# simon3dv/SLR-SFS

Hardware: AMD Instinct MI355X
Metric: synthesised frames/sec at 768x1280 N=60 (higher is better)
Workload: dtype f32 (convs: fp32 in/out/accumulate, operands 2 x f16 splits = 22 bits; all-fp32: fps_fp32_convs); 1 GPU; C3 baseline pipeline, 768x1280, N=60, random weights; parallelism=1 GPU, no collective, collective_bytes_received_per_rank_per_clip=0

## Files before the change

### slr-sfs_amd/csrc/conv.hip

```cpp
#include "slr_common.hpp"

#include <string.h>

#include <atomic>
#include <mutex>
#include <type_traits>

namespace slr {

typedef _Float16 h8 __attribute__((ext_vector_type(8)));
typedef float f16v __attribute__((ext_vector_type(16)));

constexpr int CV_W = 32, CV_H = 8;
constexpr int CV_HW = CV_W + 2, CV_HH = CV_H + 2;
constexpr int CV_NPX = CV_HW * CV_HH;
constexpr int CV_THREADS = 256;
constexpr float CV_XSCALE = 64.0f;
constexpr int CV_MAXCIN = 1024;

enum { PRE_NONE = 0, PRE_BN = 1, PRE_BN_MASK = 2, PRE_BN_NONZERO = 3 };

struct ConvArgs {
    const float *in;
    const h8 *w;
    float *out;
    int N, Cin, Cout, H, W, tiles_x, nchunk;
    float unscale;
    float xscale;
    int pre;
    const float *pre_scale, *pre_shift;
    const float *mask;
    const float *bias;
    int partial;
    float mask_scale, winsize;
    const float *residual, *next_scale, *next_shift;
    float *um_out;
    int out_b8;
    int res_b8;
    unsigned *sat;
#ifdef SLR_TRACE
    long long *trace;
#endif
    int wino_groups;
    const float *skip_in;
    const h8 *skip_w;
    const float *skip_bias;
    int skip_cin, skip_nchunk;
    float skip_unscale;
    float *pool_row, *pool_col;
    int tiles_y, resample;
    float *skip_out;
};

__host__ __device__ inline int conv_cout_tile(int Cout) { return Cout > 64 ? 128 : (Cout > 32 ? 64 : 32); }
__host__ __device__ inline int conv_cout_pad(int Cout) { const int t = conv_cout_tile(Cout); return (Cout + t - 1) / t * t; }
__host__ __device__ inline int conv_cin_pad(int Cin) { return (Cin + 15) / 16 * 16; }

}
#include "conv_few.hpp"
namespace slr {

constexpr int CV_FSTR = 352;
constexpr int CV_KSTR = 260;
template <int CPW, int WCO, bool PRE, bool INB8, bool F32 = false, bool SKIP = false, bool POOL = false, bool UPS = false>
__global__ __launch_bounds__(CV_THREADS, 2) void conv3x3_split_kernel(ConvArgs a) {
    constexpr int WPX = 4 / WCO, PT = CV_H / WPX;
    static_assert(!(POOL || UPS) || (SKIP && WCO == 4 && !(POOL && UPS)), "the resampling epilogues: a wave holds all 8 rows of its channel tile");
    static_assert(!F32 || CPW == 1, "the fp32 rung runs one 32-channel tile per wave");
    static_assert(!SKIP || (CPW == 1 && INB8), "the skip phase: one tile per wave, channel-blocked main input");
    constexpr int XRAW = F32 ? 2 * 16 * CV_FSTR * 4 : 2 * 2 * 2 * CV_NPX * 16, XSKIP = !SKIP ? 0 : SLR_CONV_SKIP_FILL * (F32 ? 16 * CV_KSTR * 4 : 2 * 2 * 256 * 16);
    __shared__ __attribute__((aligned(16))) unsigned char xraw[XRAW > XSKIP ? XRAW : XSKIP];
    h8 (*xs)[2][2][CV_NPX] = reinterpret_cast<h8 (*)[2][2][CV_NPX]>(xraw);
    float (*xf)[16][CV_FSTR] = reinterpret_cast<float (*)[16][CV_FSTR]>(xraw);
    __shared__ float mpl[CV_NPX];
    __shared__ float mplB[2][CV_NPX - 256];
    __shared__ float4 pss4[2][CV_MAXCIN / 4];
    const int tid = threadIdx.x, lane = tid & 63;
    const int wave = __builtin_amdgcn_readfirstlane(tid >> 6);
    const int wc = wave % WCO, wp = wave / WCO;
    const int tx = blockIdx.x % a.tiles_x, ty = blockIdx.x / a.tiles_x;
    const int x0 = tx * CV_W, y0 = ty * CV_H;
    const int n = blockIdx.z;
    const int cot0 = (blockIdx.y * WCO + wc) * CPW;
    const int HW = a.H * a.W;
    const int nchunk = a.nchunk;
    const int cmax = a.Cin - 1;
    const float *inb = a.in + (size_t)n * a.Cin * HW;
    const int pre = a.pre;

    if (PRE) {
        float *pssw = reinterpret_cast<float *>(&pss4[0][0]);
        for (int i = tid; i < nchunk * 16; i += CV_THREADS) {
            pssw[i] = i < a.Cin ? a.pre_scale[i] * (F32 ? 1.0f : a.xscale) : 0.0f;
            pssw[CV_MAXCIN + i] = i < a.Cin ? a.pre_shift[i] * (F32 ? 1.0f : a.xscale) : 0.0f;
        }
    }

    const int gB = tid >= 84 ? 1 : 0;
    const int pB = 256 + tid - 84 * gB;
    const bool liveB = tid < 168;
    bool okA, okB;
    int offA, offB;
    {
        const int pr = tid / CV_HW, pc = tid - pr * CV_HW;
        const int gy = y0 - 1 + pr, gx = x0 - 1 + pc;
        okA = (gy >= 0) & (gy < a.H) & (gx >= 0) & (gx < a.W);
        offA = okA ? gy * a.W + gx : 0;
    }
    {
        const int pr = pB / CV_HW, pc = pB - pr * CV_HW;
        const int gy = y0 - 1 + pr, gx = x0 - 1 + pc;
        okB = liveB & (gy >= 0) & (gy < a.H) & (gx >= 0) & (gx < a.W);
        offB = okB ? gy * a.W + gx : 0;
    }
    const float unit = (PRE || F32) ? 1.0f : a.xscale;
    const float mvA = (a.mask && okA) ? a.mask[(size_t)n * HW + offA] : 0.0f;
    const float mvB = (a.mask && okB) ? a.mask[(size_t)n * HW + offB] : 0.0f;
    if (a.mask) {
        mpl[tid] = mvA;
        if (tid < CV_NPX - 256) mpl[256 + tid] = mvB;
    }
    const float mA = okA ? (pre == PRE_BN_MASK ? mvA : unit) : 0.0f;
    const float mB = okB ? (pre == PRE_BN_MASK ? mvB : unit) : 0.0f;
    float cnt[3] = {0.0f, 0.0f, 0.0f};
    const bool nonzero_mask = pre == PRE_BN_NONZERO;
    const int c8max = (a.Cin >> 3) - 1;
    auto load_round = [&](auto R, int c, float (&st)[8]) {
        if (INB8) {
            const int grp = min(c * 2 + (R.value < 2 ? R.value : gB), c8max);
            const float4 *q = reinterpret_cast<const float4 *>(inb) + ((size_t)grp * HW + (unsigned)(R.value < 2 ? offA : offB)) * 2;
            const float4 u = q[0], v = q[1];
            st[0] = u.x; st[1] = u.y; st[2] = u.z; st[3] = u.w;
            st[4] = v.x; st[5] = v.y; st[6] = v.z; st[7] = v.w;
            return;
        }
#pragma unroll
        for (int j = 0; j < 8; ++j) {
            if (R.value < 2) {
                const float *pl = inb + (size_t)min(c * 16 + R.value * 8 + j, cmax) * HW;
                st[j] = pl[(unsigned)offA];
            } else {
                st[j] = inb[(unsigned)(min(c * 16 + gB * 8 + j, cmax) * HW + offB)];
            }
        }
    };
    struct Stage { int cb; float mk0, fresh, cnt; h8 hi, lo; float f[F32 ? 8 : 1]; };
    unsigned long long sat = 0ull;
    const float *pss = reinterpret_cast<const float *>(&pss4[0][0]);
    auto stage_begin = [&](auto R, int c, Stage &g) {
        g.cb = c * 16 + (R.value < 2 ? R.value * 8 : gB * 8);
        g.mk0 = R.value < 2 ? mA : mB;
        g.cnt = 0.0f;
    };
    auto stage_value = [&](int j, Stage &g, const float (&st)[8], const float *psc = nullptr, const float *psh = nullptr) {
        const float x = st[j];
        float v;
        if (PRE) {
            const float mk = (nonzero_mask & (x == 0.0f)) ? 0.0f : g.mk0;
            v = fmaxf(x * (psc ? psc[j] : pss[g.cb + j]) - (psh ? psh[j] : pss[CV_MAXCIN + g.cb + j]), 0.0f) * mk;
            g.cnt += (g.cb + j <= cmax) ? mk : 0.0f;
        } else if (F32) {
            v = g.mk0 != 0.0f ? x : 0.0f;
        } else {
            v = x * g.mk0;
        }
        if (F32) { g.f[j] = v; return; }
// ... 185 lines not shown
#pragma unroll
            for (int ct = 0; ct < CPW; ++ct) {
                a_cur[ct][0] = a_nxt[ct][0]; a_cur[ct][1] = a_nxt[ct][1];
                if (DEEP) { a_nxt[ct][0] = a_nx2[ct][0]; a_nxt[ct][1] = a_nx2[ct][1]; }
            }
        }
        __syncthreads();
    }

    if (pre == PRE_BN_NONZERO) {
        mpl[tid] = cnt[0] + cnt[1];
        if (liveB) mplB[gB][pB - 256] = cnt[2];
        __syncthreads();
        if (tid < CV_NPX - 256) mpl[256 + tid] = mplB[0][tid] + mplB[1][tid];
    }
    __syncthreads();

    if constexpr (SKIP) {
        constexpr int SK = SLR_CONV_SKIP_FILL;
        static_assert(SK * (F32 ? 16 * CV_KSTR * 4 : 2 * 2 * 256 * 16) <= (int)sizeof(xraw), "skip fills live in the staging buffers");
        h8 (*xk)[2][2][256] = reinterpret_cast<h8 (*)[2][2][256]>(xraw);
        float (*xkf)[16][CV_KSTR] = reinterpret_cast<float (*)[16][CV_KSTR]>(xraw);
        const int ns = a.skip_nchunk, sc8max = (a.skip_cin >> 3) - 1;
        const int spr = tid >> 5, spc = tid & 31;
        const bool sok = (y0 + spr < a.H) & (x0 + spc < a.W);
        const float smk = sok ? a.xscale : 0.0f;
        const float4 *sq = reinterpret_cast<const float4 *>(a.skip_in + (size_t)n * a.skip_cin * HW) + (size_t)(sok ? (y0 + spr) * a.W + x0 + spc : 0) * 2;
        float4 sv[SK][4];
        auto sload = [&](int s0) {
#pragma unroll
            for (int k = 0; k < SK; ++k)
#pragma unroll
                for (int g = 0; g < 2; ++g) {
                    const float4 *q = sq + (size_t)min(min(s0 + k, ns - 1) * 2 + g, sc8max) * HW * 2;
                    sv[k][2 * g] = q[0];
                    sv[k][2 * g + 1] = q[1];
                }
        };
        auto sstore = [&]() {
#pragma unroll
            for (int k = 0; k < SK; ++k)
#pragma unroll
                for (int g = 0; g < 2; ++g) {
                    const float x8[8] = {sv[k][2 * g].x, sv[k][2 * g].y, sv[k][2 * g].z, sv[k][2 * g].w,
                                         sv[k][2 * g + 1].x, sv[k][2 * g + 1].y, sv[k][2 * g + 1].z, sv[k][2 * g + 1].w};
                    if constexpr (F32) {
#pragma unroll
                        for (int j = 0; j < 8; ++j) xkf[k][8 * g + j][tid] = x8[j] * smk;
                        continue;
                    }
                    h8 hi, lo;
#pragma unroll
                    for (int j = 0; j < 8; ++j) {
                        const float v = __builtin_amdgcn_fmed3f(x8[j] * smk, -65472.0f, 65472.0f);
                        sat |= __ballot(fabsf(v) >= 65472.0f);
                        const _Float16 h = (_Float16)v;
                        hi[j] = h;
                        lo[j] = (_Float16)(v - (float)h);
                    }
                    xk[k][0][g][tid] = hi;
                    xk[k][1][g][tid] = lo;
                }
        };
        sload(0);
        {
            const bool partial = a.partial != 0, has_bias = a.bias != nullptr;
            const float unscale = a.unscale, rescale = 1.0f / a.skip_unscale;
            const float mscale = a.mask_scale, winsize = a.winsize;
            float eb[16];
#pragma unroll
            for (int r = 0; r < 16; ++r) eb[r] = has_bias ? a.bias[min(cot0 * 32 + (r & 3) + 8 * (r >> 2) + 4 * (lane >> 5), a.Cout - 1)] : 0.0f;
#pragma unroll
            for (int pt = 0; pt < PT; ++pt) {
                if (partial) {
                    float box = 0.0f;
#pragma unroll
                    for (int dy = 0; dy < 3; ++dy)
#pragma unroll
                        for (int dx = 0; dx < 3; ++dx) box += mpl[(wp * PT + pt + dy) * CV_HW + (lane & 31) + dx];
                    const float u = box * mscale;
                    const float um = F32 ? clamp01_nan(u) : fminf(fmaxf(u, 0.0f), 1.0f);
                    const float ratio = (1.0f / (u + 1e-8f)) * winsize * um;
                    const int oy = y0 + wp * PT + pt, ox = x0 + (lane & 31);
                    if (ox < a.W && oy < a.H && a.um_out && blockIdx.y == 0 && wc == 0 && lane < 32)
                        a.um_out[(size_t)n * HW + (size_t)oy * a.W + ox] = um;
#pragma unroll
                    for (int r = 0; r < 16; ++r) acc[0][pt][r] = (((acc[0][pt][r] * unscale) * ratio + eb[r]) * um) * rescale;
                } else {
#pragma unroll
                    for (int r = 0; r < 16; ++r) acc[0][pt][r] = (acc[0][pt][r] * unscale + eb[r]) * rescale;
                }
            }
        }
        const h8 *swbase = a.skip_w + (size_t)cot0 * ((size_t)ns * 128);
        for (int s0 = 0; s0 < ns; s0 += SK) {
            sstore();
            h8 sa[SK][2];
#pragma unroll
            for (int k = 0; k < SK; ++k) {
                const h8 *q = swbase + (size_t)min(s0 + k, ns - 1) * 128;
                if (F32) { sa[k][0] = q[2u * (unsigned)lane]; sa[k][1] = q[2u * (unsigned)lane + 1u]; continue; }
                sa[k][0] = q[(unsigned)lane]; sa[k][1] = q[(unsigned)lane + 64u];
            }
            __syncthreads();
            sload(s0 + SK);
            __builtin_amdgcn_sched_barrier(0);
#pragma unroll
            for (int k = 0; k < SK; ++k) {
                if (s0 + k >= ns) break;
                if constexpr (F32) {
                    typedef float f8v __attribute__((ext_vector_type(8)));
                    union AW { h8 h[2]; f8v f; } aw;
                    aw.h[0] = sa[k][0]; aw.h[1] = sa[k][1];
#pragma unroll
                    for (int kp = 0; kp < 8; ++kp) {
                        float bv[PT];
#pragma unroll
                        for (int kk = 0; kk < PT; ++kk) bv[kk] = xkf[k][kp + 8 * (lane >> 5)][(wp * PT + kk) * 32 + (lane & 31)];
#pragma unroll
                        for (int kk = 0; kk < PT; ++kk) acc[0][kk] = __builtin_amdgcn_mfma_f32_32x32x2f32(aw.f[kp], bv[kk], acc[0][kk], 0, 0, 0);
                    }
                    continue;
                }
                const h8 *xh = &xk[k][0][lane >> 5][0], *xl = &xk[k][1][lane >> 5][0];
                constexpr int PB = PT > 4 ? 4 : PT, NB = PT / PB;
#pragma unroll
                for (int hb = 0; hb < NB; ++hb) {
                    h8 bh[PB], bl[PB];
#pragma unroll
                    for (int kk = 0; kk < PB; ++kk) {
                        const int p = (wp * PT + hb * PB + kk) * 32 + (lane & 31);
                        bh[kk] = xh[p];
                        bl[kk] = xl[p];
                    }
#pragma unroll
                    for (int part = 0; part < 3; ++part)
#pragma unroll
                        for (int kk = 0; kk < PB; ++kk)
                            acc[0][hb * PB + kk] = __builtin_amdgcn_mfma_f32_32x32x16_f16(part == 0 ? sa[k][1] : sa[k][0], part == 1 ? bl[kk] : bh[kk],
                                                                                          acc[0][hb * PB + kk], 0, 0, 0);
                }
            }
            __syncthreads();
        }
    }

    if (!F32 && a.sat && sat != 0ull && lane == 0) atomicAdd(a.sat, 1u);

    if constexpr (POOL) {
        const float unscale = a.skip_unscale;
        const int ox = x0 + bcol;
        const bool xin = ox < a.W;
        const int OH = (a.H - 1) / 2 + 1, OW = (a.W - 1) / 2 + 1, C8 = a.Cout >> 3;
        float sb[16];
#pragma unroll
        for (int r = 0; r < 16; ++r) sb[r] = a.skip_bias ? a.skip_bias[min(cot0 * 32 + (r & 3) + 8 * (r >> 2) + 4 * bgrp, a.Cout - 1)] : 0.0f;
#pragma unroll
        for (int pt = 0; pt < PT; ++pt) {
            const bool ok = xin & (y0 + pt < a.H);
#pragma unroll
            for (int r = 0; r < 16; ++r) acc[0][pt][r] = ok ? acc[0][pt][r] * unscale + sb[r] : 0.0f;
        }
#pragma unroll
        for (int q = 0; q < 4; ++q) {
            const int c8 = cot0 * 4 + q;
            if (c8 * 8 + 4 * bgrp >= a.Cout) continue;
            if (xin && y0 + 7 < a.H) {
                float *rb = a.pool_row + ((((size_t)n * a.tiles_y + ty) * C8 + c8) * a.W + ox) * 8 + 4 * bgrp;
// ... 65 lines not shown
            }
        }
#pragma unroll
        for (int pt = 1; pt < PT; ++pt)
            if (y0 + pt >= a.H) {
#pragma unroll
                for (int r = 0; r < 16; ++r) acc[0][pt][r] = acc[0][pt - 1][r];
            }
#pragma unroll
        for (int q = 0; q < 4; ++q) {
            const int c8 = cot0 * 4 + q;
            float hE[PT][4], hO[PT][4];
#pragma unroll
            for (int pt = 0; pt < PT; ++pt)
#pragma unroll
                for (int e = 0; e < 4; ++e) {
                    const float v = acc[0][pt][4 * q + e];
                    const float left = __shfl_up(v, 1, 32), rgt = __shfl_down(v, 1, 32);
                    hE[pt][e] = 0.25f * left + 0.75f * v;
                    hO[pt][e] = 0.75f * v + 0.25f * (rclamp ? v : rgt);
                }
            if (!xin || c8 * 8 + 4 * bgrp >= a.Cout) continue;
            float *ob = a.out + (((size_t)n * C8 + c8) * OH * OW + (size_t)(2 * y0) * OW + 2 * ox) * 8 + 4 * bgrp;
#pragma unroll
            for (int hr = 1; hr < 2 * PT - 1; ++hr) {
                const int ra = (hr & 1) ? hr >> 1 : (hr >> 1) - 1, rb = ra + 1;
                const float l0 = (hr & 1) ? 0.75f : 0.25f, l1 = (hr & 1) ? 0.25f : 0.75f;
                if (y0 + (hr >> 1) >= a.H) continue;
                float *orow = ob + (size_t)hr * OW * 8;
                if (bcol > 0)
                    *reinterpret_cast<float4 *>(orow) = make_float4(l0 * hE[ra][0] + l1 * hE[rb][0], l0 * hE[ra][1] + l1 * hE[rb][1],
                                                                    l0 * hE[ra][2] + l1 * hE[rb][2], l0 * hE[ra][3] + l1 * hE[rb][3]);
                if (bcol < 31)
                    *reinterpret_cast<float4 *>(orow + 8) = make_float4(l0 * hO[ra][0] + l1 * hO[rb][0], l0 * hO[ra][1] + l1 * hO[rb][1],
                                                                        l0 * hO[ra][2] + l1 * hO[rb][2], l0 * hO[ra][3] + l1 * hO[rb][3]);
            }
        }
        return;
    }

    const float *ebias = SKIP ? a.skip_bias : a.bias;
    const bool partial = !SKIP && a.partial != 0, has_bias = ebias != nullptr, has_res = a.residual != nullptr,
               has_next = !SKIP && a.next_scale != nullptr;
    float *outp = a.out;
    const bool vec = !a.out_b8 && (a.W % 4 == 0) && (x0 + CV_W <= a.W) &&
                     !(((uintptr_t)a.out | (uintptr_t)a.residual) & 15);
    constexpr int SCR_STRIDE = 36;
    float *scr = reinterpret_cast<float *>(xraw) + wave * (32 * SCR_STRIDE);
    const int ox = x0 + bcol;
    const bool xin_img = ox < a.W;
    const int cout1 = a.Cout - 1;
    const float mscale = a.mask_scale, winsize = a.winsize, unscale = SKIP ? a.skip_unscale : a.unscale;
#pragma unroll
    for (int ct = 0; ct < CPW; ++ct) {
        int co[16];
#pragma unroll
        for (int r = 0; r < 16; ++r) co[r] = (cot0 + ct) * 32 + (r & 3) + 8 * (r >> 2) + 4 * bgrp;
        float eb[16], esc[16], esh[16];
        if (has_bias) {
#pragma unroll
            for (int r = 0; r < 16; ++r) eb[r] = ebias[min(co[r], cout1)];
        }
        if (has_next) {
#pragma unroll
            for (int r = 0; r < 16; ++r) { esc[r] = a.next_scale[min(co[r], cout1)]; esh[r] = a.next_shift[min(co[r], cout1)]; }
        }
#pragma unroll
        for (int pt = 0; pt < PT; ++pt) {
            const int oy = y0 + wp * PT + pt;
            const bool ok = xin_img & (oy < a.H);
            const size_t pix = ok ? (size_t)oy * a.W + ox : 0;
            float o[16];
#pragma unroll
            for (int r = 0; r < 16; ++r) o[r] = acc[ct][pt][r] * unscale;
            if (partial) {
                float box = 0.0f;
#pragma unroll
                for (int dy = 0; dy < 3; ++dy)
#pragma unroll
                    for (int dx = 0; dx < 3; ++dx) box += mpl[(wp * PT + pt + dy) * CV_HW + bcol + dx];
                const float u = box * mscale;
                const float um = F32 ? clamp01_nan(u) : fminf(fmaxf(u, 0.0f), 1.0f);
                const float ratio = (1.0f / (u + 1e-8f)) * winsize * um;
                if (ok && a.um_out && ct == 0 && blockIdx.y == 0 && wc == 0 && bgrp == 0)
                    a.um_out[(size_t)n * HW + pix] = um;
#pragma unroll
                for (int r = 0; r < 16; ++r) o[r] = (o[r] * ratio + eb[r]) * um;
                if (has_res && !vec && !a.out_b8) {
                    float rv[16];
#pragma unroll
                    for (int r = 0; r < 16; ++r) rv[r] = a.residual[((size_t)n * a.Cout + min(co[r], cout1)) * HW + pix];
#pragma unroll
                    for (int r = 0; r < 16; ++r) o[r] += rv[r];
                }
                if (has_next) {
#pragma unroll
                    for (int r = 0; r < 16; ++r) o[r] = fmaxf(o[r] * esc[r] - esh[r], 0.0f) * um;
                }
            } else {
                if (has_bias) {
#pragma unroll
                    for (int r = 0; r < 16; ++r) o[r] += eb[r];
                }
                if (has_res && !vec && !a.out_b8) {
                    float rv[16];
#pragma unroll
                    for (int r = 0; r < 16; ++r) rv[r] = a.residual[((size_t)n * a.Cout + min(co[r], cout1)) * HW + pix];
#pragma unroll
                    for (int r = 0; r < 16; ++r) o[r] += rv[r];
                }
            }
            if (a.out_b8) {
#pragma unroll
                for (int q = 0; q < 4; ++q) {
                    const int c8 = (cot0 + ct) * 4 + q;
                    const bool live = ok && c8 * 8 + 4 * bgrp < a.Cout;
                    const size_t bidx = (((size_t)n * (a.Cout >> 3) + (live ? c8 : 0)) * HW + pix) * 8 + 4 * bgrp;
                    float4 v = make_float4(o[4 * q], o[4 * q + 1], o[4 * q + 2], o[4 * q + 3]);
                    if (has_res) {
                        float4 rv;
                        if (a.res_b8) {
                            rv = *reinterpret_cast<const float4 *>(&a.residual[bidx]);
                        } else {
                            const size_t ridx = ((size_t)n * a.Cout + (live ? c8 * 8 + 4 * bgrp : 0)) * HW + pix;
                            rv = make_float4(a.residual[ridx], a.residual[ridx + HW], a.residual[ridx + 2 * (size_t)HW], a.residual[ridx + 3 * (size_t)HW]);
                        }
                        v.x += rv.x; v.y += rv.y; v.z += rv.z; v.w += rv.w;
                    }
                    if (live) *reinterpret_cast<float4 *>(&outp[bidx]) = v;
                }
            } else if (vec) {
#pragma unroll
                for (int r = 0; r < 16; ++r) scr[((r & 3) + 8 * (r >> 2) + 4 * bgrp) * SCR_STRIDE + bcol] = o[r];
                __builtin_amdgcn_wave_barrier();
                const int quad = lane & 7;
                float4 v[4], rv[4];
#pragma unroll
                for (int k = 0; k < 4; ++k) v[k] = *reinterpret_cast<const float4 *>(&scr[((lane >> 3) + 8 * k) * SCR_STRIDE + quad * 4]);
                __builtin_amdgcn_wave_barrier();
                const bool rowok = oy < a.H;
                size_t vidx[4];
#pragma unroll
                for (int k = 0; k < 4; ++k) {
                    const int cv = min((cot0 + ct) * 32 + (lane >> 3) + 8 * k, cout1);
                    vidx[k] = ((size_t)n * a.Cout + cv) * HW + (rowok ? (size_t)oy * a.W + x0 + quad * 4 : 0);
                }
                if (has_res) {
#pragma unroll
                    for (int k = 0; k < 4; ++k) rv[k] = *reinterpret_cast<const float4 *>(&a.residual[vidx[k]]);
#pragma unroll
                    for (int k = 0; k < 4; ++k) { v[k].x += rv[k].x; v[k].y += rv[k].y; v[k].z += rv[k].z; v[k].w += rv[k].w; }
                }
#pragma unroll
                for (int k = 0; k < 4; ++k)
                    if (rowok && (cot0 + ct) * 32 + (lane >> 3) + 8 * k <= cout1) *reinterpret_cast<float4 *>(&outp[vidx[k]]) = v[k];
            } else {
#pragma unroll
                for (int r = 0; r < 16; ++r)
                    if (ok && co[r] <= cout1) outp[((size_t)n * a.Cout + co[r]) * HW + pix] = o[r];
            }
        }
    }
}

constexpr int C1_TILES = 1;
template <int NCT, bool INB8, bool F32 = false>
__global__ __launch_bounds__(256) void conv1x1_split_kernel(const float *__restrict__ in, const h8 *__restrict__ w,
                                                            const float *__restrict__ bias, float *__restrict__ out,
                                                            int Cin, int Cout, int HW, int nchunk, float unscale, float xscale,
                                                            int out_b8, unsigned *__restrict__ sat_count) {
    const int lane = threadIdx.x & 63;
    const int wave = __builtin_amdgcn_readfirstlane(threadIdx.x >> 6);
    const int n = blockIdx.z;
    const int cot0 = blockIdx.y * NCT;
    const int pcol = lane & 31, grp = lane >> 5;
    const int p0 = ((blockIdx.x * 4 + wave) * C1_TILES) * 32 + pcol;
    const int cmax = Cin - 1;
    const int gend = C1_TILES * nchunk;
    const float *inb = in + (size_t)n * Cin * HW;
    auto load_x = [&](float (&x)[8], int g) {
        g = min(g, gend - 1);
        const int t = g / nchunk, c = g - t * nchunk;
        const int p = p0 + t * 32;
        const unsigned poff = p < HW ? p : 0;
        if (INB8) {
            const float4 *q4 = reinterpret_cast<const float4 *>(inb) + ((size_t)min(c * 2 + grp, (Cin >> 3) - 1) * HW + poff) * 2;
            const float4 u = q4[0], v = q4[1];
            x[0] = u.x; x[1] = u.y; x[2] = u.z; x[3] = u.w; x[4] = v.x; x[5] = v.y; x[6] = v.z; x[7] = v.w;
            return;
        }
#pragma unroll
        for (int j = 0; j < 8; ++j) x[j] = inb[(size_t)min(c * 16 + grp * 8 + j, cmax) * HW + poff];
    };
    const h8 *wb = w + (size_t)cot0 * nchunk * 128 + lane;
    auto load_a = [&](h8 (&d)[NCT][2], int g) {
        const int c = g % nchunk;
#pragma unroll
        for (int t = 0; t < NCT; ++t) {
            const h8 *q = wb + ((size_t)t * nchunk + c) * 128;
            if (F32) { d[t][0] = q[lane]; d[t][1] = q[lane + 1]; continue; }
            d[t][0] = q[0];
            d[t][1] = q[64];
        }
    };
    const int cout1 = Cout - 1;
    const bool has_bias = bias != nullptr;
    const float *bp = has_bias ? bias : in;
    f16v acc[NCT];
    float x0[8], x1[8], x2[8];
    h8 a_cur[NCT][2], a_nxt[NCT][2];
    bool sat = false;
    load_x(x0, 0);
    load_a(a_cur, 0);
    load_x(x1, 1);
    for (int tile = 0, g = 0; tile < C1_TILES; ++tile) {
        const int p = p0 + tile * 32;
        const bool ok = p < HW;
        const float okf = ok ? xscale : 0.0f;
#pragma unroll
        for (int t = 0; t < NCT; ++t)
#pragma unroll
            for (int r = 0; r < 16; ++r) acc[t][r] = 0.0f;
        for (int c = 0; c < nchunk; ++c, ++g) {
            load_a(a_nxt, g + 1);
            load_x(x2, g + 2);
            __builtin_amdgcn_sched_barrier(0);
            if constexpr (F32) {
                typedef float f8v __attribute__((ext_vector_type(8)));
                const float ok1 = ok ? 1.0f : 0.0f;
#pragma unroll
                for (int kp = 0; kp < 8; ++kp)
#pragma unroll
                    for (int t = 0; t < NCT; ++t) {
                        union AW { h8 h[2]; f8v f; } aw;
                        aw.h[0] = a_cur[t][0]; aw.h[1] = a_cur[t][1];
                        acc[t] = __builtin_amdgcn_mfma_f32_32x32x2f32(aw.f[kp], x0[kp] * ok1, acc[t], 0, 0, 0);
                    }
#pragma unroll
                for (int j = 0; j < 8; ++j) { x0[j] = x1[j]; x1[j] = x2[j]; }
#pragma unroll
                for (int t = 0; t < NCT; ++t) { a_cur[t][0] = a_nxt[t][0]; a_cur[t][1] = a_nxt[t][1]; }
                continue;
// ... 500 lines not shown
        SLR_CHECK_ARG(!sb8 && !pool, "layout flags");
        SLR_CHECK_ARG(sk->w && a.Cout <= CF_MAXCO && (layout & SLR_CONV_IN_B8) && !((uintptr_t)sk->w & 15),
                      "the skip output needs Cout <= 4, a channel-blocked input and 16-byte aligned [Cin][4] weights");
        SLR_CHECK_ARG(a.pre != PRE_BN_NONZERO, "the skip output goes with an explicit mask");
        a.skip_w = (const h8 *)sk->w; a.skip_bias = sk->bias; a.skip_out = sk->skip_out;
        return 0;
    }
    SLR_CHECK_ARG(sk->in && sk->w, "null pointer");
    SLR_CHECK_ARG(!(layout & SLR_CONV_WINO), "no fused skip branch in the Winograd kernel");
    SLR_CHECK_ARG(!(layout & SLR_CONV_F32) || (conv_cout_tile(a.Cout) == 128 && sk->wscale == 1.0f),
                  "the fused skip branch on the fp32 rung: more than 64 output channels, skip_wscale = 1");
    SLR_CHECK_ARG((layout & SLR_CONV_IN_B8) && a.Cout > CF_MAXCO, "the fused skip branch needs a channel-blocked main input and more than 4 output channels");
    SLR_CHECK_ARG(sk->cin > 0 && (long long)sk->cin * a.H * a.W < (1LL << 31) && sk->wscale > 0.0f, "skip sizes");
    SLR_CHECK_ARG(sb8 && sk->cin % 8 == 0 && !((uintptr_t)sk->in & 15), "the fused skip branch reads a channel-blocked skip input (SLR_CONV_SKIP_B8): skip_cin % 8 == 0, 16-byte aligned");
    SLR_CHECK_ARG(!a.residual && !a.next_scale, "the fused skip branch replaces the residual; no next-BN fusion with it");
    a.skip_in = sk->in; a.skip_w = (const h8 *)sk->w; a.skip_bias = sk->bias;
    a.skip_cin = sk->cin; a.skip_nchunk = conv_cin_pad(sk->cin) / 16;
    a.skip_unscale = 1.0f / (xscale * sk->wscale);
    if (pool) {
        SLR_CHECK_ARG(!(up && (layout_in & SLR_CONV_POOL_OUT)), "SLR_CONV_POOL_OUT and SLR_CONV_UP_OUT are exclusive");
        SLR_CHECK_ARG(a.out_b8 && conv_cout_tile(a.Cout) == 128, "the resampling epilogues need a channel-blocked output and more than 64 output channels");
        SLR_CHECK_ARG(!up || (long long)a.N * a.Cout * a.H * a.W < (1LL << 38), "sizes");
        SLR_CHECK_ARG(sk->pool_ws && !((uintptr_t)sk->pool_ws & 15) && sk->pool_ws_bytes >= conv_pool_ws_bytes(a.N, a.Cout, a.H, a.W, up),
                      "pool_ws: slr_conv_pool_ws_bytes / slr_conv_up_ws_bytes, 16-byte aligned");
        a.tiles_y = (a.H + CV_H - 1) / CV_H;
        a.resample = up ? 2 : 1;
        a.pool_row = (float *)sk->pool_ws;
        a.pool_col = a.pool_row + (size_t)a.N * a.Cout * a.tiles_y * a.W * (up ? 2 : 1);
    }
    return 0;
}

template <int WCO, bool PRE, bool B8, bool F32, bool SKIP, bool POOL, bool UPS>
static constexpr bool conv_split_built() {
    return !(WCO == 4 && PRE && !B8) && (B8 || !SKIP) && (!(POOL || UPS) || (SKIP && WCO == 4 && !(POOL && UPS))) &&
           !(F32 && SKIP && WCO != 4);
}

static int conv_launch(ConvArgs &a, float wscale, float xscale, int layout, hipStream_t st) {
    const bool in_b8 = (layout & SLR_CONV_IN_B8) != 0, f32 = (layout & SLR_CONV_F32) != 0, wino = (layout & SLR_CONV_WINO) != 0;
    const bool pre = a.pre != PRE_NONE;
    if (int e = check_xscale(xscale)) return e;
    SLR_CHECK_ARG(!f32 || (wscale == 1.0f && xscale == 1.0f), "the fp32 rung takes no operand scales (wscale = xscale = 1)");
    SLR_CHECK_ARG(!wino || (f32 && a.Cout > CF_MAXCO), "SLR_CONV_WINO goes with SLR_CONV_F32 and more than 4 output channels");
    SLR_CHECK_ARG(!wino || !pre || a.Cin <= WN_MAXCIN, "SLR_CONV_WINO with a prologue supports Cin <= 256");
    if (wino) {
        a.tiles_x = (a.W + WN_BW - 1) / WN_BW;
        a.nchunk = conv_cin_pad(a.Cin) / 16;
        a.xscale = 1.0f; a.unscale = 1.0f;
        const int blocks = a.tiles_x * ((a.H + WN_BH - 1) / WN_BH), ngrp = wino_cout_pad(a.Cout) / 64;
        const dim3 grid((blocks + WN_SLICE - 1) / WN_SLICE * WN_SLICE * ngrp, 1, a.N);
        a.wino_groups = ngrp;
#ifdef SLR_TRACE
        a.trace = g_trace;
#endif
        if (int e = dispatch([&](auto pre_, auto b8) {
                static LdsOptIn attr;
                if (int e = lds_opt_in((const void *)conv3x3_wino_kernel<pre_, b8>, (int)WN_LDS_BYTES, attr)) return e;
                hipLaunchKernelGGL((conv3x3_wino_kernel<pre_, b8>), grid, dim3(WN_THREADS), WN_LDS_BYTES, st, a);
                return 0;
            }, pre, in_b8)) return e;
        SLR_CHECK_LAUNCH();
        return 0;
    }
    if (a.Cout <= CF_MAXCO) {
        const dim3 grid(((a.W + CF_BW - 1) / CF_BW) * ((a.H + CF_BH - 1) / CF_BH), 1, a.N);
        if (int e = dispatch_int<1, 2, 3, 4>(a.Cout, [&](auto nco) {
                return dispatch([&](auto pre_, auto b8, auto skp) {
                    if constexpr (b8 || !skp) hipLaunchKernelGGL((conv3x3_few_kernel<nco, pre_, b8, skp>), grid, dim3(CF_THREADS), 0, st, a);
                    else return conv_not_built();
                    return 0;
                }, pre, in_b8, a.skip_out != nullptr);
            })) return e;
        SLR_CHECK_LAUNCH();
        return 0;
    }
    a.tiles_x = (a.W + CV_W - 1) / CV_W;
    a.nchunk = conv_cin_pad(a.Cin) / 16;
    a.xscale = xscale;
    a.unscale = 1.0f / (xscale * wscale);
    if (int e = sat_counter(&a.sat)) return e;
    int ct = conv_cout_tile(a.Cout);
    if (ct == 128 && pre && !in_b8) ct = 64;
    const dim3 grid(a.tiles_x * ((a.H + CV_H - 1) / CV_H), conv_cout_pad(a.Cout) / ct, a.N);
    if (int e = dispatch_int<4, 2, 1>(ct / 32, [&](auto wco) {
            return dispatch([&](auto pre_, auto b8, auto f32_, auto skip, auto pool, auto ups) {
                if constexpr (conv_split_built<wco, pre_, b8, f32_, skip, pool, ups>())
                    hipLaunchKernelGGL((conv3x3_split_kernel<1, wco, pre_, b8, f32_, skip, pool, ups>), grid, dim3(CV_THREADS), 0, st, a);
                else return conv_not_built();
                return 0;
            }, pre, in_b8, f32, a.skip_in != nullptr, a.resample == 1, a.resample == 2);
        })) return e;
    SLR_CHECK_LAUNCH();
    if (a.resample == 2) {
        const int items = 2 * a.tiles_y * 2 * a.W + 2 * a.tiles_x * 2 * a.H;
        hipLaunchKernelGGL(upsample_fix_kernel, dim3((items + 255) / 256, a.N * (a.Cout >> 3)), dim3(256), 0, st, a.out, (const float *)a.pool_row,
                           (const float *)a.pool_col, a.Cout >> 3, a.H, a.W, a.tiles_x, a.tiles_y);
        SLR_CHECK_LAUNCH();
    } else if (a.resample == 1) {
        const int OH = (a.H - 1) / 2 + 1, OW = (a.W - 1) / 2 + 1;
        const int items = (a.tiles_y - 1) * OW + (a.tiles_x - 1) * OH;
        if (items > 0) {
            hipLaunchKernelGGL(pool_fix_kernel, dim3((items + 255) / 256, a.N * (a.Cout >> 3)), dim3(256), 0, st, a.out, (const float *)a.pool_row,
                               (const float *)a.pool_col, a.Cout >> 3, a.H, a.W, a.tiles_x, a.tiles_y);
            SLR_CHECK_LAUNCH();
        }
    }
    return 0;
}

static int conv3x3_run(bool partial, const float *x, const float *pre_scale, const float *pre_shift, const float *mask,
                       const void *wsplit, float wscale, float xscale, const float *bias, const float *residual,
                       const float *next_scale, const float *next_shift, float *out, float *um_out,
                       int N, int Cin, int Cout, int H, int W, const SkipOp *sk, int layout, void *stream) {
    SLR_CHECK_ARG(x && wsplit && (bias || !partial) && out, "null pointer");
    if (int e = conv_check_layout(layout, x, out, Cin, Cout, residual, partial && !mask)) return e;
    SLR_CHECK_ARG(!pre_scale == !pre_shift, "pre_scale / pre_shift go together");
    SLR_CHECK_ARG(!pre_scale || Cin <= CV_MAXCIN, "prologue supports Cin <= 1024");
    SLR_CHECK_ARG(!partial || mask || pre_scale, "mask = NULL (derived from x != 0) needs the raw input, i.e. pre_scale / pre_shift");
    SLR_CHECK_ARG(!next_scale == !next_shift, "next_scale / next_shift go together");
    SLR_CHECK_ARG(!(residual && next_scale), "residual and next-BN fusion are exclusive");
    if (int e = conv_check_dims(N, Cin, Cout, H, W)) return e;
    ConvArgs a = {};
    a.in = x; a.w = (const h8 *)wsplit; a.bias = bias; a.out = out;
    a.N = N; a.Cin = Cin; a.Cout = Cout; a.H = H; a.W = W;
    a.pre = !pre_scale ? PRE_NONE : !partial ? PRE_BN : mask ? PRE_BN_MASK : PRE_BN_NONZERO;
    a.pre_scale = pre_scale; a.pre_shift = pre_shift; a.mask = mask;
    if (partial) {
        a.partial = 1;
        a.mask_scale = mask ? (float)Cin : 1.0f;
        a.winsize = (float)Cin * 9.0f;
    }
    a.residual = residual; a.next_scale = next_scale; a.next_shift = next_shift; a.um_out = um_out;
    a.out_b8 = (layout & SLR_CONV_OUT_B8) != 0;
    a.res_b8 = (layout & SLR_CONV_RES_B8) != 0;
    if (int e = conv_set_skip(a, sk, xscale, layout)) return e;
    return conv_launch(a, wscale, xscale, layout, (hipStream_t)stream);
}

SLR_EXPORT int slr_conv3x3_forward(const float *in, const void *wsplit, const float *bias, const float *residual,
                                   float *out, int N, int Cin, int Cout, int H, int W, float wscale, float xscale,
                                   const float *pre_scale, const float *pre_shift, int layout, void *stream) {
    return conv3x3_run(false, in, pre_scale, pre_shift, nullptr, wsplit, wscale, xscale, bias, residual, nullptr, nullptr, out, nullptr,
                       N, Cin, Cout, H, W, nullptr, layout, stream);
}

SLR_EXPORT int slr_conv3x3_forward_skip(const float *in, const void *wsplit, const float *bias, float *out,
                                        int N, int Cin, int Cout, int H, int W, float wscale, float xscale,
                                        const float *pre_scale, const float *pre_shift,
                                        const float *skip_in, const void *skip_wsplit, const float *skip_bias, int skip_cin, float skip_wscale,
                                        void *pool_ws, size_t pool_ws_bytes, int layout, void *stream) {
    const SkipOp sk = {skip_in, skip_wsplit, skip_bias, skip_cin, skip_wscale, pool_ws, pool_ws_bytes, nullptr};
    return conv3x3_run(false, in, pre_scale, pre_shift, nullptr, wsplit, wscale, xscale, bias, nullptr, nullptr, nullptr, out, nullptr,
                       N, Cin, Cout, H, W, &sk, layout, stream);
}

SLR_EXPORT int slr_conv3x3_forward_skipout(const float *in, const void *wsplit, const float *bias, const float *residual, float *out,
                                           int N, int Cin, int Cout, int H, int W, float wscale, float xscale,
                                           const float *pre_scale, const float *pre_shift,
                                           const float *skip_w4, const float *skip_bias, float *skip_out, int layout, void *stream) {
    SLR_CHECK_ARG(skip_w4 && skip_out, "null pointer");
    const SkipOp sk = {nullptr, skip_w4, skip_bias, 0, 1.0f, nullptr, 0, skip_out};
    return conv3x3_run(false, in, pre_scale, pre_shift, nullptr, wsplit, wscale, xscale, bias, residual, nullptr, nullptr, out, nullptr,
                       N, Cin, Cout, H, W, &sk, layout, stream);
}

SLR_EXPORT int slr_pconv3x3_forward(const float *x, const float *pre_scale, const float *pre_shift, const float *mask,
// ... 28 lines not shown
```

### slr-sfs_amd/csrc/slr_tuning.hpp

```cpp
#pragma once

#define SLR_TILE_H 8
#define SLR_EPT_ONE 2
#define SLR_EPT_TWO 3

#define SLR_STORE_AUX 2
#define SLR_WAVES_SCAN 4
#define SLR_KREG_TWO 6
#define SLR_LMAX 16
#define SLR_HEAVY_SLACK 24
#define SLR_HEAVY_MAX 4
#define SLR_BAL_SLACK 24
#define SLR_XCD_GROUP 4
#define SLR_BATCH_INTERLEAVE 1

#define SLR_PLAN_HEAVY 6

#define SLR_CSPLIT_MAX 4
#define SLR_CSPLIT_SLOTS 512
#define SLR_SCAN_DEFER_AT 896
#define SLR_SINK_PIECES 33
#define SLR_SINK_TASKS 16
#define SLR_SINK_POOL_MB 64
#define SLR_SINK_ENT_MB 16
#define SLR_SINK_GROUPS 8
#define SLR_SINK_GRID 512
#define SLR_WAVES_SINK_DET 4
#define SLR_SCAN_MAX_TILES 1024

#define SLR_ROW_CAP 256
#define SLR_ROWBIN_R 2
#define SLR_CLIP_MAXB 16
#define SLR_CLIP_ALIGNED 0
#define SLR_CLIP_HEAVY 0
#define SLR_WAVES_CLIP 4
#define SLR_ROWBIN_CLIP_R 4
#define SLR_ROW_CB_CLIP 4
#define SLR_ROW_CB 3
#define SLR_WAVES_ROWS 6
#define SLR_KREG_ROWS 4
#define SLR_ROWS_PLAN_PER 4
#define SLR_ROWS_FILL 7
#define SLR_EPT_DEFER 4
#define SLR_ROWS_GROUP 2
#define SLR_FRONT_END -1

#define SLR_GRAD_U 4
#define SLR_BLEND_U 4
#define SLR_GRAD_TU 4
#define SLR_GRAD_BOX 4096
#define SLR_GRAD_BENT 2
#define SLR_GRAD_STRIPS 2
#define SLR_GRAD_WAVES 4
#define SLR_GRAD_SLOTS 1024
#define SLR_GRAD_GROUPS_MAX 4
#define SLR_GRAD_GROUPS_MIN 2

#define SLR_CONV_SKIP_FILL 3

#define SLR_CONV_DEEP_STAGE 1

#define SLR_WGRAD_SLOTS 512
#define SLR_WGRAD_WS_MB 32
#ifdef __cplusplus
inline long long slr_wgrad_auto_splits(long long chunks, long long channel_tiles, long long bytes_per_slab) {
    long long s = (SLR_WGRAD_SLOTS + channel_tiles - 1) / channel_tiles;
    const long long cap = ((long long)SLR_WGRAD_WS_MB << 20) / bytes_per_slab;
    if (s > cap) s = cap;
    if (s > chunks) s = chunks;
    return s < 1 ? 1 : s;
}
#endif

#define SLR_WGRAD1_SLOTS 256
#define SLR_WGRAD1_WS_MB 8
#ifdef __cplusplus
inline long long slr_wgrad1x1_auto_splits(long long chunks, long long channel_tiles, long long bytes_per_slab) {
    long long s = (SLR_WGRAD1_SLOTS + channel_tiles - 1) / channel_tiles;
    const long long cap = ((long long)SLR_WGRAD1_WS_MB << 20) / bytes_per_slab;
    if (s > cap) s = cap;
    if (s > chunks) s = chunks;
    return s < 1 ? 1 : s;
}
#endif


#ifdef SLR_TUNING_OVERRIDE
#include SLR_TUNING_OVERRIDE
#endif
```

Measured before the change: 187.7 frames/s.

## Remap conv3x3 block order into XCD-aware tile groups and stream output stores

Replaces the linear blockIdx-to-tile mapping with a grouped order. Blocks covering a small 2x2 group of spatial tiles, and all their output-channel blocks, are assigned round-robin so each group lands on one XCD. The goal is to reuse input halos and tiles in each XCD's L2 instead of spreading neighbours across chiplets. Output and uncertainty-mask stores become nontemporal so write-once results do not evict reusable input lines. The grid is padded to a multiple of 8 groups, which adds some early-exiting blocks, and nontemporal stores could hurt if a following kernel reads the outputs from cache.

```diff
diff --git a/slr-sfs_amd/csrc/conv.hip b/slr-sfs_amd/csrc/conv.hip
--- a/slr-sfs_amd/csrc/conv.hip
+++ b/slr-sfs_amd/csrc/conv.hip
@@ -1,4 +1,5 @@
 #include "slr_common.hpp"
+#include "conv_order.hpp"
 
 #include <string.h>
 
@@ -10,6 +11,10 @@
 
 typedef _Float16 h8 __attribute__((ext_vector_type(8)));
 typedef float f16v __attribute__((ext_vector_type(16)));
+typedef float f4v __attribute__((ext_vector_type(4)));
+
+__device__ __forceinline__ void stream_store(float *p, float4 v) { __builtin_nontemporal_store(f4v{v.x, v.y, v.z, v.w}, reinterpret_cast<f4v *>(p)); }
+__device__ __forceinline__ void stream_store(float *p, float v) { __builtin_nontemporal_store(v, p); }
 
 constexpr int CV_W = 32, CV_H = 8;
 constexpr int CV_HW = CV_W + 2, CV_HH = CV_H + 2;
@@ -49,6 +54,7 @@
     float skip_unscale;
     float *pool_row, *pool_col;
     int tiles_y, resample;
+    int nblock;
     float *skip_out;
 };
 
@@ -78,10 +84,12 @@
     const int tid = threadIdx.x, lane = tid & 63;
     const int wave = __builtin_amdgcn_readfirstlane(tid >> 6);
     const int wc = wave % WCO, wp = wave / WCO;
-    const int tx = blockIdx.x % a.tiles_x, ty = blockIdx.x / a.tiles_x;
+    ConvItem item;
+    if (!conv_order_item(blockIdx.x, a.tiles_x, a.tiles_y, a.nblock, SLR_CONV_ORDER_G, SLR_CONV_ORDER_ROWS, item)) return;
+    const int tx = item.tx, ty = item.ty;
     const int x0 = tx * CV_W, y0 = ty * CV_H;
     const int n = blockIdx.z;
-    const int cot0 = (blockIdx.y * WCO + wc) * CPW;
+    const int cot0 = (item.block * WCO + wc) * CPW;
     const int HW = a.H * a.W;
     const int nchunk = a.nchunk;
     const int cmax = a.Cin - 1;
@@ -433,8 +441,8 @@
                     const float um = F32 ? clamp01_nan(u) : fminf(fmaxf(u, 0.0f), 1.0f);
                     const float ratio = (1.0f / (u + 1e-8f)) * winsize * um;
                     const int oy = y0 + wp * PT + pt, ox = x0 + (lane & 31);
-                    if (ox < a.W && oy < a.H && a.um_out && blockIdx.y == 0 && wc == 0 && lane < 32)
-                        a.um_out[(size_t)n * HW + (size_t)oy * a.W + ox] = um;
+                    if (ox < a.W && oy < a.H && a.um_out && item.block == 0 && wc == 0 && lane < 32)
+                        stream_store(&a.um_out[(size_t)n * HW + (size_t)oy * a.W + ox], um);
 #pragma unroll
                     for (int r = 0; r < 16; ++r) acc[0][pt][r] = (((acc[0][pt][r] * unscale) * ratio + eb[r]) * um) * rescale;
                 } else {
@@ -666,8 +674,8 @@
                 const float u = box * mscale;
                 const float um = F32 ? clamp01_nan(u) : fminf(fmaxf(u, 0.0f), 1.0f);
                 const float ratio = (1.0f / (u + 1e-8f)) * winsize * um;
-                if (ok && a.um_out && ct == 0 && blockIdx.y == 0 && wc == 0 && bgrp == 0)
-                    a.um_out[(size_t)n * HW + pix] = um;
+                if (ok && a.um_out && ct == 0 && item.block == 0 && wc == 0 && bgrp == 0)
+                    stream_store(&a.um_out[(size_t)n * HW + pix], um);
 #pragma unroll
                 for (int r = 0; r < 16; ++r) o[r] = (o[r] * ratio + eb[r]) * um;
                 if (has_res && !vec && !a.out_b8) {
@@ -711,7 +719,7 @@
                         }
                         v.x += rv.x; v.y += rv.y; v.z += rv.z; v.w += rv.w;
                     }
-                    if (live) *reinterpret_cast<float4 *>(&outp[bidx]) = v;
+                    if (live) stream_store(&outp[bidx], v);
                 }
             } else if (vec) {
 #pragma unroll
@@ -737,11 +745,11 @@
                 }
 #pragma unroll
                 for (int k = 0; k < 4; ++k)
-                    if (rowok && (cot0 + ct) * 32 + (lane >> 3) + 8 * k <= cout1) *reinterpret_cast<float4 *>(&outp[vidx[k]]) = v[k];
+                    if (rowok && (cot0 + ct) * 32 + (lane >> 3) + 8 * k <= cout1) stream_store(&outp[vidx[k]], v[k]);
             } else {
 #pragma unroll
                 for (int r = 0; r < 16; ++r)
-                    if (ok && co[r] <= cout1) outp[((size_t)n * a.Cout + co[r]) * HW + pix] = o[r];
+                    if (ok && co[r] <= cout1) stream_store(&outp[((size_t)n * a.Cout + co[r]) * HW + pix], o[r]);
             }
         }
     }
@@ -1408,7 +1416,9 @@
     if (int e = sat_counter(&a.sat)) return e;
     int ct = conv_cout_tile(a.Cout);
     if (ct == 128 && pre && !in_b8) ct = 64;
-    const dim3 grid(a.tiles_x * ((a.H + CV_H - 1) / CV_H), conv_cout_pad(a.Cout) / ct, a.N);
+    a.tiles_y = (a.H + CV_H - 1) / CV_H;
+    a.nblock = conv_cout_pad(a.Cout) / ct;
+    const dim3 grid(conv_order_grid(a.tiles_x, a.tiles_y, a.nblock, SLR_CONV_ORDER_G, SLR_CONV_ORDER_ROWS), 1, a.N);
     if (int e = dispatch_int<4, 2, 1>(ct / 32, [&](auto wco) {
             return dispatch([&](auto pre_, auto b8, auto f32_, auto skip, auto pool, auto ups) {
                 if constexpr (conv_split_built<wco, pre_, b8, f32_, skip, pool, ups>())
diff --git a/slr-sfs_amd/csrc/conv_order.hpp b/slr-sfs_amd/csrc/conv_order.hpp
--- /dev/null
+++ b/slr-sfs_amd/csrc/conv_order.hpp
@@ -0,0 +1,37 @@
+#pragma once
+
+#ifndef __host__
+#define __host__
+#define __device__
+#endif
+
+namespace slr {
+
+constexpr int CONV_ORDER_XCDS = 8;
+
+struct ConvItem { int tx, ty, block; };
+
+__host__ __device__ inline int conv_order_groups(int tiles_x, int tiles_y, int G, int rows) {
+    const int gcols = G / rows;
+    return ((tiles_x + gcols - 1) / gcols) * ((tiles_y + rows - 1) / rows);
+}
+
+__host__ __device__ inline int conv_order_grid(int tiles_x, int tiles_y, int nblock, int G, int rows) {
+    const int groups = conv_order_groups(tiles_x, tiles_y, G, rows);
+    return (groups + CONV_ORDER_XCDS - 1) / CONV_ORDER_XCDS * CONV_ORDER_XCDS * G * nblock;
+}
+
+__host__ __device__ inline bool conv_order_item(int b, int tiles_x, int tiles_y, int nblock, int G, int rows, ConvItem &it) {
+    const int per_slice = CONV_ORDER_XCDS * G * nblock;
+    const int slice = b / per_slice, r = b - slice * per_slice;
+    const int group = slice * CONV_ORDER_XCDS + r % CONV_ORDER_XCDS, k = r / CONV_ORDER_XCDS;
+    const int t = k / nblock;
+    const int gcols = G / rows, gpb = (tiles_x + gcols - 1) / gcols;
+    const int band = group / gpb, gc = group - band * gpb;
+    it.block = k - t * nblock;
+    it.tx = gc * gcols + t / rows;
+    it.ty = band * rows + t % rows;
+    return it.tx < tiles_x && it.ty < tiles_y;
+}
+
+}
diff --git a/slr-sfs_amd/csrc/slr_tuning.hpp b/slr-sfs_amd/csrc/slr_tuning.hpp
--- a/slr-sfs_amd/csrc/slr_tuning.hpp
+++ b/slr-sfs_amd/csrc/slr_tuning.hpp
@@ -60,6 +60,9 @@
 
 #define SLR_CONV_DEEP_STAGE 1
 
+#define SLR_CONV_ORDER_G 4
+#define SLR_CONV_ORDER_ROWS 2
+
 #define SLR_WGRAD_SLOTS 512
 #define SLR_WGRAD_WS_MB 32
 #ifdef __cplusplus
```

Measured after the change: 189.2 frames/s, median of 6. About the same (+0.8%).
